# LIONS-EPFL/LEAF

Hardware: NVIDIA B200
Metric: leaf_candidates_scored_per_sec (higher is better)
Workload: dtype bf16

## Files before the change

include/leaf_b200.h:

```cpp
#ifndef LEAF_B200_H_
#define LEAF_B200_H_

#include <stdint.h>

#ifdef __cplusplus
extern "C" {
#endif

typedef enum {
  LEAF_OK = 0,
  LEAF_ERR_INVALID = -1,
  LEAF_ERR_CUDA = -2,
  LEAF_ERR_STATE = -3,
  LEAF_ERR_UNSUPPORTED = -4
} leaf_status_t;

typedef struct leaf_engine* leaf_handle_t;

enum { LEAF_ACT_GELU_ERF = 0, LEAF_ACT_QUICK_GELU = 1 };
enum { LEAF_OBJ_L2 = 0, LEAF_OBJ_NEGL2 = 1, LEAF_OBJ_SIM = 2, LEAF_OBJ_DISSIM = 3 };
enum { LEAF_CTX = 77, LEAF_SOT = 49406, LEAF_EOT = 49407, LEAF_VOCAB = 49408, LEAF_N_MERGES = 48894 };
enum { LEAF_MAX_CAPTION_BYTES = 1000, LEAF_MAX_CAPTION_BYTES_LONG = 3560 };

typedef struct {
// ... 68 lines not shown

typedef void (*leaf_backward_hook_t)(int32_t layer, void* user);
int leaf_set_backward_hook(leaf_handle_t h, leaf_backward_hook_t fn, void* user);
int leaf_set_sm_budget(leaf_handle_t h, int32_t n_sms);
int leaf_set_deterministic(leaf_handle_t h, int32_t on);

int leaf_adamw(leaf_handle_t h, float* params, const float* grads, float* exp_avg, float* exp_avg_sq, int64_t n,
               int64_t n_nodecay, float lr, float beta1, float beta2, float eps, float weight_decay, int32_t step,
               float grad_scale, void* stream);
int leaf_sumsq(leaf_handle_t h, const float* g, int64_t n, float* out, void* stream);
int leaf_scale(leaf_handle_t h, float* g, int64_t n, float s, void* stream);

int leaf_gemm_bf16(leaf_handle_t h, const void* A, const void* Bt, const float* bias, void* C,
                   int32_t M, int32_t N, int32_t K, int32_t epilogue, int32_t act, const int32_t* m_dev,
                   void* stream);
int leaf_gemm_bf16_mn(leaf_handle_t h, const void* A, const void* B, const float* bias, void* C, int32_t M, int32_t N,
                      int32_t K, int32_t epilogue, int32_t a_mn, void* stream);
int leaf_test_layernorm(leaf_handle_t h, const float* x, int32_t rows, const float* gamma, const float* beta, void* y,
                        void* stream);
int leaf_test_attention(leaf_handle_t h, const void* qkv, const int32_t* meta, int32_t N, void* out, void* stream);
int leaf_test_attention_bwd(leaf_handle_t h, const void* qkv, const void* o, const float* dout, const int32_t* meta, int32_t N,
                            int32_t T, void* dqkv, void* stream);
int leaf_set_prune_last(leaf_handle_t h, int32_t on);
int64_t leaf_launch_count(leaf_handle_t h, int32_t reset);
int64_t leaf_last_rows(leaf_handle_t h);
int leaf_set_timing(leaf_handle_t h, int32_t on);
double leaf_timing_ms(leaf_handle_t h, int32_t which, int32_t* launches);

#ifdef __cplusplus
}
// ... 3 lines not shown
```

leaf_b200/_native.py:

```python
import ctypes
import os

HERE = os.path.dirname(os.path.abspath(__file__))
LIB_PATH = os.environ.get("LEAF_B200_LIB") or os.path.join(HERE, "lib", "libleaf_b200.so")

c_int, c_void_p, c_float, c_i64 = ctypes.c_int32, ctypes.c_void_p, ctypes.c_float, ctypes.c_int64


class LeafCfg(ctypes.Structure):
    _fields_ = [("width", c_int), ("layers", c_int), ("heads", c_int), ("embed_dim", c_int), ("activation", c_int),
                ("ln_eps", c_float)]


class LeafLayerPtrs(ctypes.Structure):
    _fields_ = [(k, c_void_p) for k in (
        "ln1_w", "ln1_b", "in_proj_w", "in_proj_b", "q_w", "k_w", "v_w", "q_b", "k_b", "v_b", "out_w", "out_b",
        "ln2_w", "ln2_b", "fc1_w", "fc1_b", "fc2_w", "fc2_b")]


class LeafWeightPtrs(ctypes.Structure):
    _fields_ = [("token_embedding", c_void_p), ("positional_embedding", c_void_p), ("lnf_w", c_void_p),
                ("lnf_b", c_void_p), ("text_projection", c_void_p), ("projection_is_ew", c_int),
                ("layers", ctypes.POINTER(LeafLayerPtrs))]

# ... 17 lines not shown
    "leaf_encode": (c_int, [c_void_p, c_void_p, c_void_p, c_void_p, c_int, c_int, c_int, c_int, c_int, c_void_p, c_void_p]),
    "leaf_score": (c_int, [c_void_p, c_void_p, c_void_p, c_int, c_int, c_int, c_void_p, c_void_p, c_void_p, c_void_p]),
    "leaf_topk": (c_int, [c_void_p, c_void_p, c_void_p, c_int, c_int, c_void_p, c_void_p, c_void_p]),
    "leaf_train_reserve": (c_int, [c_void_p, c_int]),
    "leaf_forward_train": (c_int, [c_void_p, c_void_p, c_void_p, c_int, c_void_p, c_int, c_int, ctypes.POINTER(c_i64), c_void_p]),
    "leaf_backward": (c_int, [c_void_p, c_i64, c_void_p, c_int, ctypes.POINTER(LeafWeightPtrs), c_void_p]),
    "leaf_set_backward_hook": (c_int, [c_void_p, c_void_p, c_void_p]),
    "leaf_set_sm_budget": (c_int, [c_void_p, c_int]),
    "leaf_set_deterministic": (c_int, [c_void_p, c_int]),
    "leaf_adamw": (c_int, [c_void_p, c_void_p, c_void_p, c_void_p, c_void_p, c_i64, c_i64, ctypes.c_float, ctypes.c_float,
                           ctypes.c_float, ctypes.c_float, ctypes.c_float, c_int, ctypes.c_float, c_void_p]),
    "leaf_sumsq": (c_int, [c_void_p, c_void_p, c_i64, c_void_p, c_void_p]),
    "leaf_scale": (c_int, [c_void_p, c_void_p, c_i64, ctypes.c_float, c_void_p]),
    "leaf_gemm_bf16": (c_int, [c_void_p, c_void_p, c_void_p, c_void_p, c_void_p, c_int, c_int, c_int, c_int, c_int,
                               c_void_p, c_void_p]),
    "leaf_gemm_bf16_mn": (c_int, [c_void_p, c_void_p, c_void_p, c_void_p, c_void_p, c_int, c_int, c_int, c_int, c_int, c_void_p]),
    "leaf_test_layernorm": (c_int, [c_void_p, c_void_p, c_int, c_void_p, c_void_p, c_void_p, c_void_p]),
    "leaf_test_attention": (c_int, [c_void_p, c_void_p, c_void_p, c_int, c_void_p, c_void_p]),
    "leaf_test_attention_bwd": (c_int, [c_void_p, c_void_p, c_void_p, c_void_p, c_void_p, c_int, c_int, c_void_p, c_void_p]),
    "leaf_set_prune_last": (c_int, [c_void_p, c_int]),
    "leaf_launch_count": (c_i64, [c_void_p, c_int]),
    "leaf_last_rows": (c_i64, [c_void_p]),
    "leaf_set_timing": (c_int, [c_void_p, c_int]),
    "leaf_timing_ms": (ctypes.c_double, [c_void_p, c_int, ctypes.POINTER(c_int)]),
}

BACKWARD_HOOK = ctypes.CFUNCTYPE(None, c_int, c_void_p)

_lib = None

# ... 24 lines not shown
```

leaf_b200/csrc/engine.cu:

```cuda
#include <cuda.h>
#include <cuda_bf16.h>
#include <cuda_runtime.h>
#include <stdarg.h>
#include <stdint.h>
#include <stdio.h>
#include <stdlib.h>
#include <string.h>

#include <algorithm>
#include <map>
#include <string>
#include <tuple>
#include <vector>

#include "../../include/leaf_b200.h"
#include "gemm2_sm100.cuh"
#include "gemm_sm100.cuh"
#include "k1_tables_host.h"
#include "constrain_kernel.cuh"
#include "k1_tokenize.cuh"
#include "tower_kernels.cuh"
#include "attention2.cuh"
#include "train_kernels.cuh"

// ... 139 lines not shown
  cuuint64_t dims[2] = {static_cast<cuuint64_t>(mn_cols), static_cast<cuuint64_t>(k_rows)};
  cuuint64_t strides[1] = {static_cast<cuuint64_t>(pitch) * 2};
  cuuint32_t box[2] = {64, 64};
  cuuint32_t estr[2] = {1, 1};
  CUtensorMap m;
  CUresult r = e->encode_tiled(&m, CU_TENSOR_MAP_DATA_TYPE_BFLOAT16, 2, const_cast<void*>(ptr), dims, strides, box, estr,
                               CU_TENSOR_MAP_INTERLEAVE_NONE, CU_TENSOR_MAP_SWIZZLE_128B,
                               CU_TENSOR_MAP_L2_PROMOTION_L2_256B, CU_TENSOR_MAP_FLOAT_OOB_FILL_NONE);
  if (r != CUDA_SUCCESS) return fail(LEAF_ERR_CUDA, "cuTensorMapEncodeTiled (MN-major) failed (%d) rows=%ld cols=%ld", (int)r, k_rows, mn_cols);
  if (e->tmaps.size() > 4096) e->tmaps.clear();
  e->tmaps[key] = m;
  *out = m;
  return LEAF_OK;
}

static cudaEvent_t get_event(leaf_engine* e) {
  if (!e->event_pool.empty()) { cudaEvent_t ev = e->event_pool.back(); e->event_pool.pop_back(); return ev; }
  cudaEvent_t ev;
  cudaEventCreate(&ev);
  return ev;
}

struct TimedSpan {
  leaf_engine* e; cudaStream_t st; cudaEvent_t a = nullptr, b = nullptr; int cat;
  TimedSpan(leaf_engine* e_, int cat_, cudaStream_t st_) : e(e_), st(st_), cat(cat_) {
    if (e->timing) { a = get_event(e); b = get_event(e); cudaEventRecord(a, st); }
  }
  ~TimedSpan() {
    if (a) { cudaEventRecord(b, st); e->spans.push_back({a, b, cat}); }
  }
};

static int launch_gemm(leaf_engine* e, const __nv_bfloat16* A, long a_rows, const __nv_bfloat16* Bt, const float* bias,
                       void* C, int ldc, int M, int N, int K, int epi, int act, const int* m_dev, cudaStream_t st,
                       const __nv_bfloat16* delta = nullptr, int mn_major = 0, long a_pitch = 0, const float* res = nullptr,
                       void* C2 = nullptr, bool allow_split_k = false) {
  if (M <= 0 || N <= 0 || K <= 0) return fail(LEAF_ERR_INVALID, "GEMM shape %dx%dx%d", M, N, K);
  if (N % 8 != 0) return fail(LEAF_ERR_INVALID, "GEMM N (%d) must be a multiple of 8", N);
  CUtensorMap ta, tb;
  int a_box = a_rows < 128 ? static_cast<int>(a_rows) : 128;
  int b_box = N < 128 ? N : 128;
  int rc;
  if (mn_major & GEMM_A_MN) {
    if (M % 8 != 0) return fail(LEAF_ERR_INVALID, "MN-major GEMM M (%d) must be a multiple of 8", M);
    if ((rc = make_tmap_mn(e, A, K, M, a_pitch, &ta))) return rc;
    a_box = 128;
  } else if ((rc = make_tmap(e, A, a_rows, K, a_box, &ta))) return rc;
  if (mn_major & GEMM_B_MN) {
    if ((rc = make_tmap_mn(e, Bt, K, N, 0, &tb))) return rc;
    b_box = 128;
  } else if ((rc = make_tmap(e, Bt, N, K, b_box, &tb))) return rc;
  GemmParams p;
  p.mn_major = mn_major;
  p.res = res;
  p.C2 = C2;
  p.split_k = 1;
  p.ws = nullptr;
  p.cnt = nullptr;
  p.tx_bytes = static_cast<uint32_t>(a_box + b_box) * GEMM_BK * 2 * 2;
  p.M = M; p.m_dev = m_dev; p.N = N; p.K = K; p.bias = bias; p.C = C; p.ldc = ldc; p.act = act; p.delta = delta;
  const int m_tiles = (M + GEMM2_BM - 1) / GEMM2_BM, n_tiles = (N + GEMM_BN - 1) / GEMM_BN;
  long tiles = static_cast<long>(m_tiles) * n_tiles;
  const int pairs_cap = ((e->gemm_sm_budget > 0 && e->gemm_sm_budget < e->sm_count) ? e->gemm_sm_budget : e->sm_count) / 2;
  const bool det = e->deterministic && ((epi == EPI_BF16_ACTBWD && C2) || allow_split_k);
  const int split_pairs = det ? e->sm_count / 2 : pairs_cap;
  if (det) {
    if (!e->tw.det_ws) return fail(LEAF_ERR_STATE, "deterministic mode without its workspace (leaf_train_reserve)");
    p.ws = e->tw.det_ws;
    p.cnt = e->tw.det_cnt;
    if (epi == EPI_BF16_ACTBWD) {
      if (static_cast<size_t>((M + 31) / 32) * N > e->tw.det_ws_floats || static_cast<size_t>(n_tiles) * 4 > e->tw.det_cnt_ints)
// ... 5 lines not shown
    const int kblocks = (K + GEMM_BK - 1) / GEMM_BK;
    long best = ((tiles + split_pairs - 1) / split_pairs) * (kblocks + 3);
    for (int s = 2; s <= 8 && s <= kblocks; ++s) {
      const int kpb = (kblocks + s - 1) / s;
      const int s_eff = (kblocks + kpb - 1) / kpb;
      if (det && tiles * s_eff > 2L * split_pairs) continue;
      const long cost = ((tiles * s_eff + split_pairs - 1) / split_pairs) * (kpb + 3);
      if (cost < best) { best = cost; p.split_k = s_eff; }
    }
    if (det && p.split_k > 1 && (static_cast<size_t>(tiles) * p.split_k * GEMM2_BM * GEMM_BN > e->tw.det_ws_floats ||
                                 static_cast<size_t>(tiles) * 2 * EPI_WARPS > e->tw.det_cnt_ints))
      return fail(LEAF_ERR_STATE, "deterministic workspace too small for a %dx%d split-K product", M, N);
    tiles *= p.split_k;
    if (p.split_k > 1) epi = det ? EPI_F32_SPLITK_DET : EPI_F32_SPLITK;
  }
  TimedSpan span(e, (epi == EPI_F32_SPLITK || epi == EPI_F32_SPLITK_DET) ? 4 + EPI_F32_RESIDUAL :
                    (epi == EPI_BF16_ACTBWD || epi == EPI_BF16_ACTBWD_DET) ? 4 + EPI_F32 : (epi == EPI_F32_RESIDUAL && K > N) ? 8 : (epi == EPI_BF16 && K == N) ? 9 : 4 + epi, st);
  const int pairs = static_cast<int>(tiles < pairs_cap ? tiles : pairs_cap);
  cudaLaunchConfig_t cfg{};
  cfg.gridDim = dim3(2 * pairs);
  cfg.blockDim = dim3(GEMM_THREADS);
  cfg.dynamicSmemBytes = GEMM2_SMEM_BYTES;
  cfg.stream = st;
  cudaLaunchAttribute attr[2];
  attr[0].id = cudaLaunchAttributeClusterDimension;
  attr[0].val.clusterDim.x = 2; attr[0].val.clusterDim.y = 1; attr[0].val.clusterDim.z = 1;
  attr[1].id = cudaLaunchAttributeProgrammaticStreamSerialization;
  attr[1].val.programmaticStreamSerializationAllowed = 1;
  cfg.attrs = attr;
  cfg.numAttrs = e->pdl ? 2 : 1;
  switch (epi) {
    case EPI_BF16: CK(cudaLaunchKernelEx(&cfg, gemm2_bf16_tn_kernel<EPI_BF16>, ta, tb, p)); break;
    case EPI_BF16_ACT: CK(cudaLaunchKernelEx(&cfg, gemm2_bf16_tn_kernel<EPI_BF16_ACT>, ta, tb, p)); break;
    case EPI_F32_RESIDUAL: CK(cudaLaunchKernelEx(&cfg, gemm2_bf16_tn_kernel<EPI_F32_RESIDUAL>, ta, tb, p)); break;
    case EPI_F32: CK(cudaLaunchKernelEx(&cfg, gemm2_bf16_tn_kernel<EPI_F32>, ta, tb, p)); break;
    case EPI_F32_SPLITK: CK(cudaLaunchKernelEx(&cfg, gemm2_bf16_tn_kernel<EPI_F32_SPLITK>, ta, tb, p)); break;
    case EPI_BF16_ACTBWD: CK(cudaLaunchKernelEx(&cfg, gemm2_bf16_tn_kernel<EPI_BF16_ACTBWD>, ta, tb, p)); break;
    case EPI_F32_SPLITK_DET: CK(cudaLaunchKernelEx(&cfg, gemm2_bf16_tn_kernel<EPI_F32_SPLITK_DET>, ta, tb, p)); break;
    case EPI_BF16_ACTBWD_DET: CK(cudaLaunchKernelEx(&cfg, gemm2_bf16_tn_kernel<EPI_BF16_ACTBWD_DET>, ta, tb, p)); break;
    default: return fail(LEAF_ERR_INVALID, "unknown epilogue %d", epi);
  }
  e->launches++;
  CK(cudaGetLastError());
  return LEAF_OK;
}

extern "C" int leaf_create(const leaf_cfg_t* cfg, leaf_handle_t* out) {
  if (!cfg || !out) return fail(LEAF_ERR_INVALID, "null argument");
  if (cfg->width <= 0 || cfg->width % 128 != 0 || cfg->width > 2048)
    return fail(LEAF_ERR_INVALID, "width %d must be a multiple of 128 in (0, 2048]", cfg->width);
  if (cfg->heads <= 0 || cfg->width != cfg->heads * 64) return fail(LEAF_ERR_INVALID, "head_dim must be 64 (W=%d, H=%d)", cfg->width, cfg->heads);
  if (cfg->embed_dim <= 0 || cfg->embed_dim % 8 != 0) return fail(LEAF_ERR_INVALID, "embed_dim %d must be a multiple of 8", cfg->embed_dim);
  if (cfg->layers <= 0) return fail(LEAF_ERR_INVALID, "layers");
  int ndev = 0;
// ... 384 lines not shown
  if (!e || !score_a || !idx_out) return fail(LEAF_ERR_INVALID, "null argument");
  if (m <= 0 || k <= 0 || k > m) return fail(LEAF_ERR_INVALID, "top-k of m=%d, k=%d", m, k);
  const size_t smem = static_cast<size_t>(m) * 4;
  if (smem > 200 * 1024) return fail(LEAF_ERR_INVALID, "m=%d too large (max %d)", m, 200 * 1024 / 4);
  topk_kernel<<<1, 1024, smem, static_cast<cudaStream_t>(stream)>>>(score_a, score_b, m, k, idx_out, val_out);
  e->launches++;
  CK(cudaGetLastError());
  return LEAF_OK;
}

extern "C" int leaf_gemm_bf16(leaf_handle_t e, const void* A, const void* Bt, const float* bias, void* C, int32_t M, int32_t N,
                              int32_t K, int32_t epilogue, int32_t act, const int32_t* m_dev, void* stream) {
  if (!e || !A || !Bt || !C) return fail(LEAF_ERR_INVALID, "null argument");
  return launch_gemm(e, static_cast<const __nv_bfloat16*>(A), M, static_cast<const __nv_bfloat16*>(Bt), bias, C, N, M, N, K,
                     epilogue, act, m_dev, static_cast<cudaStream_t>(stream));
}

extern "C" int leaf_gemm_bf16_mn(leaf_handle_t e, const void* A, const void* B, const float* bias, void* C, int32_t M, int32_t N,
                                 int32_t K, int32_t epilogue, int32_t a_mn, void* stream) {
  if (!e || !A || !B || !C) return fail(LEAF_ERR_INVALID, "null argument");
  return launch_gemm(e, static_cast<const __nv_bfloat16*>(A), a_mn ? K : M, static_cast<const __nv_bfloat16*>(B), bias, C, N, M, N, K,
                     epilogue, 0, nullptr, static_cast<cudaStream_t>(stream), nullptr, GEMM_B_MN | (a_mn ? GEMM_A_MN : 0));
}

extern "C" int leaf_test_layernorm(leaf_handle_t e, const float* x, int32_t rows, const float* gamma, const float* beta, void* y,
                                   void* stream) {
  if (!e || !x || !gamma || !beta || !y || rows <= 0) return fail(LEAF_ERR_INVALID, "bad argument");
  return launch_layernorm(e, x, nullptr, rows, nullptr, gamma, beta, static_cast<__nv_bfloat16*>(y), static_cast<cudaStream_t>(stream));
}

// ... 469 lines not shown
```

leaf_b200/csrc/gemm2_sm100.cuh:

```cuda
#pragma once
#include "gemm_sm100.cuh"

namespace leaf {

constexpr int GEMM2_BM = 256;
constexpr int GEMM2_STAGES = 5;
constexpr uint32_t GEMM2_A_BYTES = 128 * GEMM_BK * 2;
constexpr uint32_t GEMM2_B_BYTES = 128 * GEMM_BK * 2;
constexpr uint32_t GEMM2_STAGE_BYTES = GEMM2_A_BYTES + GEMM2_B_BYTES;
constexpr uint32_t GEMM2_SMEM_BYTES = GEMM2_STAGES * GEMM2_STAGE_BYTES + EPI_WARPS * EPI_STAGE_BYTES + 1024  + 256 ;
constexpr int WARP_TMA = EPI_WARPS, WARP_MMA = EPI_WARPS + 1, WARP_TMEM = EPI_WARPS + 2;
constexpr uint32_t PEER_BIT_MASK = 0xFEFFFFFFu;

__device__ __forceinline__ uint32_t cluster_ctarank() {
  uint32_t r;
  asm volatile("mov.u32 %0, %%cluster_ctarank;" : "=r"(r));
  return r;
}
__device__ __forceinline__ bool elect_one() {
  uint32_t pred;
  asm volatile("{\n\t.reg .pred p;\n\telect.sync _|p, 0xffffffff;\n\tselp.u32 %0, 1, 0, p;\n\t}" : "=r"(pred));
  return pred != 0;
}
__device__ __forceinline__ void cluster_sync_all() {
  asm volatile("barrier.cluster.arrive.release.aligned;" ::: "memory");
// ... 19 lines not shown
      "tcgen05.mma.cta_group::2.kind::f16 [%0], %1, %2, %3, p;\n\t}"
      ::"r"(tmem_d), "l"(adesc), "l"(bdesc), "r"(idesc), "r"(accumulate)
      : "memory");
}
__device__ __forceinline__ void umma_commit_2sm(uint32_t bar) {
  asm volatile("tcgen05.commit.cta_group::2.mbarrier::arrive::one.shared::cluster.multicast::cluster.b64 [%0], %1;"
               ::"r"(bar), "h"(static_cast<uint16_t>(3)) : "memory");
}
__device__ __forceinline__ void mbar_arrive_leader(uint32_t bar_local) {
  asm volatile("mbarrier.arrive.shared::cluster.b64 _, [%0];" ::"r"(bar_local & PEER_BIT_MASK) : "memory");
}

template <int EPI>
__global__ void __launch_bounds__(GEMM_THREADS, 1)
gemm2_bf16_tn_kernel(const __grid_constant__ CUtensorMap tmap_a, const __grid_constant__ CUtensorMap tmap_b,
                     const GemmParams p) {
  extern __shared__ uint8_t smem_raw[];
  const uint32_t smem_base = (smem_u32(smem_raw) + 1023u) & ~1023u;
  const uint32_t bar_base = smem_base + GEMM2_STAGES * GEMM2_STAGE_BYTES + EPI_WARPS * EPI_STAGE_BYTES;
  auto full_bar = [&](int s) { return bar_base + 8u * s; };
  auto empty_bar = [&](int s) { return bar_base + 8u * (GEMM2_STAGES + s); };
  auto tfull_bar = [&](int s) { return bar_base + 8u * (2 * GEMM2_STAGES + s); };
  auto tempty_bar = [&](int s) { return bar_base + 8u * (2 * GEMM2_STAGES + 2 + s); };
  const uint32_t tmem_slot = bar_base + 8u * (2 * GEMM2_STAGES + 4);
  uint8_t* smem_gen = smem_raw + (smem_base - smem_u32(smem_raw));
  volatile uint32_t* tmem_slot_gen =
      reinterpret_cast<volatile uint32_t*>(smem_gen + GEMM2_STAGES * GEMM2_STAGE_BYTES + EPI_WARPS * EPI_STAGE_BYTES +
                                           8u * (2 * GEMM2_STAGES + 4));

  const int warp = threadIdx.x >> 5;
  const int lane = threadIdx.x & 31;
  const uint32_t rank = cluster_ctarank();
  const bool leader = rank == 0;
  const int pair = blockIdx.x >> 1, n_pairs = gridDim.x >> 1;
  const int M = p.m_dev ? min(*p.m_dev, p.M) : p.M;
  const int m_tiles = (M + GEMM2_BM - 1) / GEMM2_BM;
  const int n_tiles = (p.N + GEMM_BN - 1) / GEMM_BN;
  const int k_blocks = (p.K + GEMM_BK - 1) / GEMM_BK;
  const int split = ((EPI == EPI_F32_SPLITK || EPI == EPI_F32_SPLITK_DET) && p.split_k > 1) ? p.split_k : 1;
  const int kpb = (k_blocks + split - 1) / split;
  const int total_tiles = m_tiles * n_tiles * split;

  if (warp == WARP_TMA && lane == 0) {
    tma_prefetch_desc(&tmap_a);
    tma_prefetch_desc(&tmap_b);
  }
  if (warp == WARP_MMA && lane == 0) {
    for (int s = 0; s < GEMM2_STAGES; ++s) {
      mbar_init(full_bar(s), 1);
      mbar_init(empty_bar(s), 1);
    }
    for (int s = 0; s < 2; ++s) {
      mbar_init(tfull_bar(s), 1);
      mbar_init(tempty_bar(s), 2 * EPI_WARPS);
    }
    asm volatile("fence.mbarrier_init.release.cluster;" ::: "memory");
  }
  if (warp == WARP_TMEM) tmem_alloc_2sm(tmem_slot, 512);
  tc_fence_before();
  cluster_sync_all();
// ... 60 lines not shown
            umma_bf16_2sm(d_tmem, adesc + 2 * ak, bdesc + 2 * bk, idesc, 1u);
            umma_bf16_2sm(d_tmem, adesc + 3 * ak, bdesc + 3 * bk, idesc, 1u);
            umma_commit_2sm(empty_bar(stage));
            if (kb == kb1 - 1) umma_commit_2sm(tfull_bar(acc));
          }
          __syncwarp();
          if (++stage == GEMM2_STAGES) { stage = 0; phase ^= 1; }
        }
        if (++acc == 2) { acc = 0; acc_phase ^= 1; }
      }
    }
  } else if (warp < EPI_WARPS) {
    const int quad = warp & 3;
    const int part = warp >> 2;
    uint8_t* stage_buf = smem_gen + GEMM2_STAGES * GEMM2_STAGE_BYTES + warp * EPI_STAGE_BYTES;
    int acc = 0;
    uint32_t acc_phase = 0;
    for (int tile = pair; tile < total_tiles; tile += n_pairs) {
      const int mn = tile / split;
      const int m_blk = mn / n_tiles, n_blk = mn % n_tiles;
      mbar_wait(tfull_bar(acc), acc_phase);
      tc_fence_after();
      const int row0 = m_blk * GEMM2_BM + static_cast<int>(rank) * 128 + quad * 32;
#pragma unroll 1
      for (int c = 0; c < 64; c += 32) {
        const int col0 = n_blk * GEMM_BN + part * 64 + c;
        if (col0 >= p.N) break;
        ResidualRegs res;
        if (row0 < M) epilogue_load_residual<EPI>(p, res, lane, row0, col0, M);
        uint32_t v[32];
        const uint32_t taddr = tmem_base + (static_cast<uint32_t>(quad * 32) << 16) +
                               static_cast<uint32_t>(acc * GEMM_BN + part * 64 + c);
        tmem_ld32(taddr, v);
        tmem_ld_wait();
        if constexpr (EPI == EPI_F32_SPLITK_DET) {
          if (row0 < M) {
            float* w = p.ws + static_cast<size_t>(tile) * (GEMM2_BM * GEMM_BN) + ((rank * EPI_WARPS + warp) * 2 + (c >> 5)) * 1024 + lane;
#pragma unroll
            for (int j = 0; j < 32; ++j) w[j * 32] = __uint_as_float(v[j]);
          }
        } else {
          if (row0 < M) epilogue_chunk<EPI>(p, v, res, stage_buf, lane, row0, col0, M);
        }
      }
      tc_fence_before();
      __syncwarp();
      if (lane == 0) mbar_arrive_leader(tempty_bar(acc));
      if (++acc == 2) { acc = 0; acc_phase ^= 1; }
      if constexpr (EPI == EPI_F32_SPLITK_DET) {
        int* ctr = p.cnt + mn * (2 * EPI_WARPS) + rank * EPI_WARPS + warp;
// ... 41 lines not shown
          const int chunks = (M + 31) >> 5;
          if (old == chunks - 1) {
            __threadfence();
#pragma unroll 1
            for (int c = 0; c < 64; c += 32) {
              const int col = n_blk * GEMM_BN + part * 64 + c + lane;
              if (col < p.N) {
                reinterpret_cast<float*>(p.C2)[col] += ordered_sum<16>(p.ws + col, p.N, chunks);
              }
            }
            if (lane == 0) *ctr = 0;
          }
        }
      }
    }
  }

  tc_fence_before();
  cluster_sync_all();
  if (warp == WARP_TMEM) {
    tc_fence_after();
    tmem_dealloc_2sm(tmem_base, 512);
  }
}

}
```

leaf_b200/csrc/gemm_sm100.cuh:

```cuda
#pragma once
#include <cuda.h>
#include <cuda_bf16.h>
#include <cuda_runtime.h>
#include <stdint.h>

namespace leaf {

__device__ __forceinline__ void pdl_wait() { asm volatile("griddepcontrol.wait;" ::: "memory"); }
__device__ __forceinline__ void pdl_trigger() { asm volatile("griddepcontrol.launch_dependents;" ::: "memory"); }

constexpr int GEMM_BN = 256;
constexpr int GEMM_BK = 64;
constexpr int GEMM_UMMA_K = 16;

enum { EPI_BF16 = 0, EPI_BF16_ACT = 1, EPI_F32_RESIDUAL = 2, EPI_F32 = 3, EPI_F32_SPLITK = 4,
       EPI_BF16_ACTBWD = 5,
       EPI_F32_SPLITK_DET = 6, EPI_BF16_ACTBWD_DET = 7 };
enum { ACT_GELU_ERF = 0, ACT_QUICK_GELU = 1 };

struct GemmParams {
  int M;
  const int* m_dev;
  int N, K;
  const float* bias;
  void* C;
  const __nv_bfloat16* delta;
  const float* res;
  int ldc;
  int act;
  uint32_t tx_bytes;
  int mn_major;
  void* C2;
  int split_k;
  float* ws;
  int* cnt;
};
constexpr int GEMM_A_MN = 1, GEMM_B_MN = 2;
constexpr uint32_t GEMM_MN_LBO = 8192, GEMM_MN_SBO = 1024, GEMM_MN_KSTEP = 2048;

__device__ __forceinline__ uint32_t smem_u32(const void* p) {
  return static_cast<uint32_t>(__cvta_generic_to_shared(p));
}
__device__ __forceinline__ void mbar_init(uint32_t bar, uint32_t count) {
  asm volatile("mbarrier.init.shared::cta.b64 [%0], %1;" ::"r"(bar), "r"(count) : "memory");
}
__device__ __forceinline__ void mbar_arrive_expect_tx(uint32_t bar, uint32_t bytes) {
  asm volatile("mbarrier.arrive.expect_tx.shared::cta.b64 _, [%0], %1;" ::"r"(bar), "r"(bytes) : "memory");
}
__device__ __forceinline__ void mbar_arrive(uint32_t bar) {
  asm volatile("mbarrier.arrive.shared::cta.b64 _, [%0];" ::"r"(bar) : "memory");
// ... 11 lines not shown
        : "memory");
    if (done) return;
    if (it == 1024) t0 = clock64();
    if (it > 1024 && (it & 1023) == 0 && clock64() - t0 > 4000000000LL) __trap();
  }
}
__device__ __forceinline__ void tma_load_2d(uint32_t smem_dst, const CUtensorMap* tmap, uint32_t bar, int x, int y) {
  asm volatile(
      "cp.async.bulk.tensor.2d.shared::cluster.global.mbarrier::complete_tx::bytes [%0], [%1, {%3, %4}], [%2];"
      ::"r"(smem_dst), "l"(reinterpret_cast<uint64_t>(tmap)), "r"(bar), "r"(x), "r"(y)
      : "memory");
}
__device__ __forceinline__ void tma_prefetch_desc(const CUtensorMap* tmap) {
  asm volatile("prefetch.tensormap [%0];" ::"l"(reinterpret_cast<uint64_t>(tmap)) : "memory");
}
__device__ __forceinline__ void tc_fence_before() { asm volatile("tcgen05.fence::before_thread_sync;" ::: "memory"); }
__device__ __forceinline__ void tc_fence_after() { asm volatile("tcgen05.fence::after_thread_sync;" ::: "memory"); }
__device__ __forceinline__ void tmem_alloc(uint32_t smem_dst, uint32_t cols) {
  asm volatile("tcgen05.alloc.cta_group::1.sync.aligned.shared::cta.b32 [%0], %1;" ::"r"(smem_dst), "r"(cols) : "memory");
  asm volatile("tcgen05.relinquish_alloc_permit.cta_group::1.sync.aligned;" ::: "memory");
}
__device__ __forceinline__ void tmem_dealloc(uint32_t taddr, uint32_t cols) {
  asm volatile("tcgen05.dealloc.cta_group::1.sync.aligned.b32 %0, %1;" ::"r"(taddr), "r"(cols) : "memory");
}
__device__ __forceinline__ void umma_bf16(uint32_t tmem_d, uint64_t adesc, uint64_t bdesc, uint32_t idesc, uint32_t accumulate) {
  asm volatile(
      "{\n\t.reg .pred p;\n\t"
      "setp.ne.b32 p, %4, 0;\n\t"
      "tcgen05.mma.cta_group::1.kind::f16 [%0], %1, %2, %3, p;\n\t}"
      ::"r"(tmem_d), "l"(adesc), "l"(bdesc), "r"(idesc), "r"(accumulate)
// ... 72 lines not shown
__device__ __forceinline__ float quick_gelu(float x) {
  return x * fast_rcp(1.0f + fast_ex2(-1.702f * 1.4426950408889634f * x));
}
__device__ __forceinline__ float gelu_erf_grad(float x) {
  const float x2 = fminf(x * x, 36.0f);
  const float r = fmaf(x2, fmaf(x2, 0.0011236976601259265f, -0.10762115607988151f), -2.299969046114191f);
  const float cdf = fast_rcp(1.0f + fast_ex2(x * r));
  const float pdf = 0.3989422804014327f * fast_ex2(-0.5f * 1.4426950408889634f * x2);
  return fmaf(x, pdf, cdf);
}
__device__ __forceinline__ float quick_gelu_grad(float x) {
  const float s = fast_rcp(1.0f + fast_ex2(-1.702f * 1.4426950408889634f * x));
  return fmaf(1.702f * x * s, 1.0f - s, s);
}
constexpr int EPI_WARPS = 16;
constexpr int EPI_STAGE_BYTES = 32 * 80;
constexpr int GEMM_THREADS = 128 + 32 * EPI_WARPS;

struct ResidualRegs { float4 x[8]; };

template <int EPI>
__device__ __forceinline__ void epilogue_load_residual(const GemmParams& p, ResidualRegs& r, int lane, int row0, int col0, int M) {
  if (EPI != EPI_F32_RESIDUAL) return;
  const int c = lane & 3;
#pragma unroll
  for (int h = 0; h < 2; ++h) {
#pragma unroll
    for (int it = 0; it < 4; ++it) {
      const int row = row0 + it * 8 + (lane >> 2);
      const int col = col0 + h * 16 + c * 4;
      if (row < M && col < p.N)
        r.x[h * 4 + it] = *reinterpret_cast<const float4*>((p.res ? p.res : reinterpret_cast<const float*>(p.C)) + static_cast<size_t>(row) * p.ldc + col);
// ... 30 lines not shown
      pk.z = *reinterpret_cast<uint32_t*>(&t2);
      pk.w = *reinterpret_cast<uint32_t*>(&t3);
      *reinterpret_cast<uint4*>(stage + lane * 80 + q * 16) = pk;
    }
    __syncwarp();
    const bool col_ok = col0 + c * 8 < p.N;
#pragma unroll
    for (int it = 0; it < 4; ++it) {
      const int r = it * 8 + (lane >> 2);
      const uint4 pk = *reinterpret_cast<const uint4*>(stage + r * 80 + c * 16);
      if (col_ok && row0 + r < M)
        *reinterpret_cast<uint4*>(reinterpret_cast<__nv_bfloat16*>(dst) + static_cast<size_t>(row0 + r) * p.ldc + col0 + c * 8) = pk;
    }
    __syncwarp();
  };
  if (EPI == EPI_BF16_ACT) {
    if (p.C2) store_bf16(p.C2);
    if (p.act == ACT_QUICK_GELU) {
#pragma unroll
      for (int j = 0; j < 32; ++j) f[j] = quick_gelu(f[j]);
    } else {
#pragma unroll
      for (int j = 0; j < 32; ++j) f[j] = gelu_erf(f[j]);
    }
  }
  if (EPI == EPI_BF16_ACTBWD || EPI == EPI_BF16_ACTBWD_DET) {
#pragma unroll
    for (int it = 0; it < 4; ++it) {
      const int r = it * 8 + (lane >> 2);
      uint4 pk = make_uint4(0u, 0u, 0u, 0u);
      if (col0 + c * 8 < p.N && row0 + r < M)
        pk = *reinterpret_cast<const uint4*>(p.delta + static_cast<size_t>(row0 + r) * p.ldc + col0 + c * 8);
      *reinterpret_cast<uint4*>(stage + r * 80 + c * 16) = pk;
    }
    __syncwarp();
    const bool live = row0 + lane < M;
#pragma unroll
    for (int q = 0; q < 4; ++q) {
      const uint4 pk = *reinterpret_cast<const uint4*>(stage + lane * 80 + q * 16);
      const uint32_t w[4] = {pk.x, pk.y, pk.z, pk.w};
// ... 14 lines not shown
      for (int off = 16; off >= 1; off >>= 1) {
        const bool up = lane & off;
#pragma unroll
        for (int j = 0; j < off; ++j) {
          const float keep = up ? f[j + off] : f[j];
          const float send = up ? f[j] : f[j + off];
          f[j] = keep + __shfl_xor_sync(0xffffffffu, send, off);
        }
      }
      if (EPI == EPI_BF16_ACTBWD_DET) {
        if (col0 + lane < p.N) p.ws[static_cast<size_t>(row0 >> 5) * p.N + col0 + lane] = f[0];
      } else if (col0 + lane < p.N) {
        atomicAdd(reinterpret_cast<float*>(p.C2) + col0 + lane, f[0]);
      }
    }
  } else if (EPI == EPI_BF16 || EPI == EPI_BF16_ACT) {
    store_bf16(p.C);
  } else {
#pragma unroll
    for (int h = 0; h < 2; ++h) {
      uint2 dl[4];
      if (EPI == EPI_F32_RESIDUAL && p.delta) {
#pragma unroll
        for (int it = 0; it < 4; ++it) {
          const int row = row0 + it * 8 + (lane >> 2), col = col0 + h * 16 + c * 4;
          dl[it] = (row < M && col < p.N) ? *reinterpret_cast<const uint2*>(p.delta + static_cast<size_t>(row) * p.ldc + col)
                                          : make_uint2(0u, 0u);
        }
      }
#pragma unroll
      for (int q = 0; q < 4; ++q)
// ... 32 lines not shown
```

leaf_b200/engine.py:

```python
from __future__ import annotations

import ctypes
import os

import numpy as np
import torch

from . import _native
from ._native import LeafCfg, LeafLayerPtrs, LeafWeightPtrs, LeafError, check

HERE = os.path.dirname(os.path.abspath(__file__))
MERGES_BIN = os.path.join(HERE, "data", "clip_bpe_merges.bin")

CONTEXT_LENGTH = 77
OBJECTIVES = {"l2": 0, "negl2": 1, "sim": 2, "dissim": 3}
STATUS_ENTITY_DOMAIN, STATUS_NON_ASCII, STATUS_TOO_LONG = 1, 2, 4
MAX_CAPTION_BYTES = 1000
MAX_CAPTION_BYTES_LONG = 3560
MAX_CODE_POINT = 0x24F


def _ptr(t):
    return None if t is None else ctypes.c_void_p(t.data_ptr())

# ... 327 lines not shown
        val = torch.empty((k,), dtype=torch.float32, device=self.device)
        with torch.cuda.device(self.device):
            check(self._lib.leaf_topk(self._h, _ptr(score_a.contiguous()), _ptr(None if score_b is None else score_b.contiguous()), m, int(k),
                                      _ptr(idx), _ptr(val), _stream()))
        return idx, val

    def gemm(self, A, Bt, bias=None, epilogue=0, act=0, C=None, m_dev=None):
        M, K = A.shape
        N = Bt.shape[0]
        if C is None:
            C = torch.empty((M, N), dtype=torch.bfloat16 if epilogue in (0, 1) else torch.float32, device=A.device)
        with torch.cuda.device(self.device):
            check(self._lib.leaf_gemm_bf16(self._h, _ptr(A), _ptr(Bt), _ptr(bias), _ptr(C), M, N, K, epilogue, act, _ptr(m_dev), _stream()))
        return C

    def gemm_mn(self, A, B, bias=None, epilogue=3, C=None, a_mn=True):
        K, N = B.shape
        M = A.shape[1] if a_mn else A.shape[0]
        if C is None:
            C = torch.zeros((M, N), dtype=torch.bfloat16 if epilogue in (0, 1) else torch.float32, device=A.device)
        with torch.cuda.device(self.device):
            check(self._lib.leaf_gemm_bf16_mn(self._h, _ptr(A), _ptr(B), _ptr(bias), _ptr(C), M, N, K, epilogue, 1 if a_mn else 0,
                                              _stream()))
        return C

    def test_layernorm(self, x, gamma, beta):
        y = torch.empty(x.shape, dtype=torch.bfloat16, device=x.device)
        check(self._lib.leaf_test_layernorm(self._h, _ptr(x), x.shape[0], _ptr(gamma), _ptr(beta), _ptr(y), _stream()))
        return y

# ... 85 lines not shown
```

Before: 78480.

## Store GEMM epilogue outputs via TMA bulk tensor stores for act and f32 paths

```diff
diff --git a/include/leaf_b200.h b/include/leaf_b200.h
--- a/include/leaf_b200.h
+++ b/include/leaf_b200.h
@@ -106,6 +106,9 @@
 int leaf_gemm_bf16(leaf_handle_t h, const void* A, const void* Bt, const float* bias, void* C,
                    int32_t M, int32_t N, int32_t K, int32_t epilogue, int32_t act, const int32_t* m_dev,
                    void* stream);
+int leaf_gemm_bf16_ex(leaf_handle_t h, const void* A, const void* Bt, const float* bias, void* C, int32_t ldc, void* C2,
+                      const float* res, const void* delta, int32_t M, int32_t N, int32_t K, int32_t epilogue, int32_t act,
+                      const int32_t* m_dev, void* stream);
 int leaf_gemm_bf16_mn(leaf_handle_t h, const void* A, const void* B, const float* bias, void* C, int32_t M, int32_t N,
                       int32_t K, int32_t epilogue, int32_t a_mn, void* stream);
 int leaf_test_layernorm(leaf_handle_t h, const float* x, int32_t rows, const float* gamma, const float* beta, void* y,
diff --git a/leaf_b200/_native.py b/leaf_b200/_native.py
--- a/leaf_b200/_native.py
+++ b/leaf_b200/_native.py
@@ -55,6 +55,8 @@
     "leaf_scale": (c_int, [c_void_p, c_void_p, c_i64, ctypes.c_float, c_void_p]),
     "leaf_gemm_bf16": (c_int, [c_void_p, c_void_p, c_void_p, c_void_p, c_void_p, c_int, c_int, c_int, c_int, c_int,
                                c_void_p, c_void_p]),
+    "leaf_gemm_bf16_ex": (c_int, [c_void_p, c_void_p, c_void_p, c_void_p, c_void_p, c_int, c_void_p, c_void_p, c_void_p, c_int,
+                                  c_int, c_int, c_int, c_int, c_void_p, c_void_p]),
     "leaf_gemm_bf16_mn": (c_int, [c_void_p, c_void_p, c_void_p, c_void_p, c_void_p, c_int, c_int, c_int, c_int, c_int, c_void_p]),
     "leaf_test_layernorm": (c_int, [c_void_p, c_void_p, c_int, c_void_p, c_void_p, c_void_p, c_void_p]),
     "leaf_test_attention": (c_int, [c_void_p, c_void_p, c_void_p, c_int, c_void_p, c_void_p]),
diff --git a/leaf_b200/csrc/engine.cu b/leaf_b200/csrc/engine.cu
--- a/leaf_b200/csrc/engine.cu
+++ b/leaf_b200/csrc/engine.cu
@@ -177,6 +177,27 @@
   return LEAF_OK;
 }
 
+static int make_tmap_out(leaf_engine* e, const void* ptr, long rows, long cols, long pitch, int elem_bytes, CUtensorMap* out) {
+  auto key = std::make_tuple(ptr, rows, cols, static_cast<int>(0x40000000L | (static_cast<long>(elem_bytes) << 24) | pitch));
+  auto it = e->tmaps.find(key);
+  if (it != e->tmaps.end()) { *out = it->second; return LEAF_OK; }
+  if ((reinterpret_cast<uintptr_t>(ptr) & 15) || (pitch * elem_bytes) % 16 != 0 || pitch >= (1L << 24))
+    return fail(LEAF_ERR_INVALID, "GEMM output must be 16-byte aligned with a 16-byte multiple row pitch (pitch %ld)", pitch);
+  cuuint64_t dims[2] = {static_cast<cuuint64_t>(cols), static_cast<cuuint64_t>(rows)};
+  cuuint64_t strides[1] = {static_cast<cuuint64_t>(pitch) * elem_bytes};
+  cuuint32_t box[2] = {static_cast<cuuint32_t>(64 / elem_bytes), 32};
+  cuuint32_t estr[2] = {1, 1};
+  CUtensorMap m;
+  CUresult r = e->encode_tiled(&m, elem_bytes == 2 ? CU_TENSOR_MAP_DATA_TYPE_BFLOAT16 : CU_TENSOR_MAP_DATA_TYPE_FLOAT32, 2,
+                               const_cast<void*>(ptr), dims, strides, box, estr, CU_TENSOR_MAP_INTERLEAVE_NONE,
+                               CU_TENSOR_MAP_SWIZZLE_64B, CU_TENSOR_MAP_L2_PROMOTION_L2_128B, CU_TENSOR_MAP_FLOAT_OOB_FILL_NONE);
+  if (r != CUDA_SUCCESS) return fail(LEAF_ERR_CUDA, "cuTensorMapEncodeTiled (output) failed (%d) rows=%ld cols=%ld", (int)r, rows, cols);
+  if (e->tmaps.size() > 4096) e->tmaps.clear();
+  e->tmaps[key] = m;
+  *out = m;
+  return LEAF_OK;
+}
+
 static cudaEvent_t get_event(leaf_engine* e) {
   if (!e->event_pool.empty()) { cudaEvent_t ev = e->event_pool.back(); e->event_pool.pop_back(); return ev; }
   cudaEvent_t ev;
@@ -200,6 +221,15 @@
                        void* C2 = nullptr, bool allow_split_k = false) {
   if (M <= 0 || N <= 0 || K <= 0) return fail(LEAF_ERR_INVALID, "GEMM shape %dx%dx%d", M, N, K);
   if (N % 8 != 0) return fail(LEAF_ERR_INVALID, "GEMM N (%d) must be a multiple of 8", N);
+  {
+    const bool bf16_out = epi == EPI_BF16 || epi == EPI_BF16_ACT || epi == EPI_BF16_ACTBWD;
+    auto rows_aligned = [&](const void* ptr, int elem_bytes) {
+      return !ptr || ((reinterpret_cast<uintptr_t>(ptr) & 15) == 0 && (static_cast<long>(ldc) * elem_bytes) % 16 == 0);
+    };
+    if (ldc < N || !rows_aligned(C, bf16_out ? 2 : 4) || (epi == EPI_BF16_ACT && !rows_aligned(C2, 2)) ||
+        !rows_aligned(res, 4) || !rows_aligned(delta, 2))
+      return fail(LEAF_ERR_INVALID, "GEMM output rows must be 16-byte aligned (ldc %d, N %d)", ldc, N);
+  }
   CUtensorMap ta, tb;
   int a_box = a_rows < 128 ? static_cast<int>(a_rows) : 128;
   int b_box = N < 128 ? N : 128;
@@ -218,6 +248,7 @@
   p.res = res;
   p.C2 = C2;
   p.split_k = 1;
+  p.c_tma = 0;
   p.ws = nullptr;
   p.cnt = nullptr;
   p.tx_bytes = static_cast<uint32_t>(a_box + b_box) * GEMM_BK * 2 * 2;
@@ -253,6 +284,12 @@
     tiles *= p.split_k;
     if (p.split_k > 1) epi = det ? EPI_F32_SPLITK_DET : EPI_F32_SPLITK;
   }
+  CUtensorMap tc{}, tc2{};
+  if ((epi == EPI_BF16_ACT || epi == EPI_F32) && M >= 32) {
+    if ((rc = make_tmap_out(e, C, M, N, ldc, epi == EPI_F32 ? 4 : 2, &tc))) return rc;
+    if (epi == EPI_BF16_ACT && C2 && (rc = make_tmap_out(e, C2, M, N, ldc, 2, &tc2))) return rc;
+    p.c_tma = 1;
+  }
   TimedSpan span(e, (epi == EPI_F32_SPLITK || epi == EPI_F32_SPLITK_DET) ? 4 + EPI_F32_RESIDUAL :
                     (epi == EPI_BF16_ACTBWD || epi == EPI_BF16_ACTBWD_DET) ? 4 + EPI_F32 : (epi == EPI_F32_RESIDUAL && K > N) ? 8 : (epi == EPI_BF16 && K == N) ? 9 : 4 + epi, st);
   const int pairs = static_cast<int>(tiles < pairs_cap ? tiles : pairs_cap);
@@ -269,14 +306,14 @@
   cfg.attrs = attr;
   cfg.numAttrs = e->pdl ? 2 : 1;
   switch (epi) {
-    case EPI_BF16: CK(cudaLaunchKernelEx(&cfg, gemm2_bf16_tn_kernel<EPI_BF16>, ta, tb, p)); break;
-    case EPI_BF16_ACT: CK(cudaLaunchKernelEx(&cfg, gemm2_bf16_tn_kernel<EPI_BF16_ACT>, ta, tb, p)); break;
-    case EPI_F32_RESIDUAL: CK(cudaLaunchKernelEx(&cfg, gemm2_bf16_tn_kernel<EPI_F32_RESIDUAL>, ta, tb, p)); break;
-    case EPI_F32: CK(cudaLaunchKernelEx(&cfg, gemm2_bf16_tn_kernel<EPI_F32>, ta, tb, p)); break;
-    case EPI_F32_SPLITK: CK(cudaLaunchKernelEx(&cfg, gemm2_bf16_tn_kernel<EPI_F32_SPLITK>, ta, tb, p)); break;
-    case EPI_BF16_ACTBWD: CK(cudaLaunchKernelEx(&cfg, gemm2_bf16_tn_kernel<EPI_BF16_ACTBWD>, ta, tb, p)); break;
-    case EPI_F32_SPLITK_DET: CK(cudaLaunchKernelEx(&cfg, gemm2_bf16_tn_kernel<EPI_F32_SPLITK_DET>, ta, tb, p)); break;
-    case EPI_BF16_ACTBWD_DET: CK(cudaLaunchKernelEx(&cfg, gemm2_bf16_tn_kernel<EPI_BF16_ACTBWD_DET>, ta, tb, p)); break;
+    case EPI_BF16: CK(cudaLaunchKernelEx(&cfg, gemm2_bf16_tn_kernel<EPI_BF16>, ta, tb, tc, tc2, p)); break;
+    case EPI_BF16_ACT: CK(cudaLaunchKernelEx(&cfg, gemm2_bf16_tn_kernel<EPI_BF16_ACT>, ta, tb, tc, tc2, p)); break;
+    case EPI_F32_RESIDUAL: CK(cudaLaunchKernelEx(&cfg, gemm2_bf16_tn_kernel<EPI_F32_RESIDUAL>, ta, tb, tc, tc2, p)); break;
+    case EPI_F32: CK(cudaLaunchKernelEx(&cfg, gemm2_bf16_tn_kernel<EPI_F32>, ta, tb, tc, tc2, p)); break;
+    case EPI_F32_SPLITK: CK(cudaLaunchKernelEx(&cfg, gemm2_bf16_tn_kernel<EPI_F32_SPLITK>, ta, tb, tc, tc2, p)); break;
+    case EPI_BF16_ACTBWD: CK(cudaLaunchKernelEx(&cfg, gemm2_bf16_tn_kernel<EPI_BF16_ACTBWD>, ta, tb, tc, tc2, p)); break;
+    case EPI_F32_SPLITK_DET: CK(cudaLaunchKernelEx(&cfg, gemm2_bf16_tn_kernel<EPI_F32_SPLITK_DET>, ta, tb, tc, tc2, p)); break;
+    case EPI_BF16_ACTBWD_DET: CK(cudaLaunchKernelEx(&cfg, gemm2_bf16_tn_kernel<EPI_BF16_ACTBWD_DET>, ta, tb, tc, tc2, p)); break;
     default: return fail(LEAF_ERR_INVALID, "unknown epilogue %d", epi);
   }
   e->launches++;
@@ -691,6 +728,17 @@
   if (!e || !A || !Bt || !C) return fail(LEAF_ERR_INVALID, "null argument");
   return launch_gemm(e, static_cast<const __nv_bfloat16*>(A), M, static_cast<const __nv_bfloat16*>(Bt), bias, C, N, M, N, K,
                      epilogue, act, m_dev, static_cast<cudaStream_t>(stream));
+}
+
+extern "C" int leaf_gemm_bf16_ex(leaf_handle_t e, const void* A, const void* Bt, const float* bias, void* C, int32_t ldc, void* C2,
+                                 const float* res, const void* delta, int32_t M, int32_t N, int32_t K, int32_t epilogue, int32_t act,
+                                 const int32_t* m_dev, void* stream) {
+  if (!e || !A || !Bt || !C) return fail(LEAF_ERR_INVALID, "null argument");
+  if (ldc < N) return fail(LEAF_ERR_INVALID, "ldc %d < N %d", ldc, N);
+  if ((C2 && epilogue != EPI_BF16_ACT) || ((res || delta) && epilogue != EPI_F32_RESIDUAL))
+    return fail(LEAF_ERR_INVALID, "C2 goes with epilogue 1, res and delta with epilogue 2");
+  return launch_gemm(e, static_cast<const __nv_bfloat16*>(A), M, static_cast<const __nv_bfloat16*>(Bt), bias, C, ldc, M, N, K,
+                     epilogue, act, m_dev, static_cast<cudaStream_t>(stream), static_cast<const __nv_bfloat16*>(delta), 0, 0, res, C2);
 }
 
 extern "C" int leaf_gemm_bf16_mn(leaf_handle_t e, const void* A, const void* B, const float* bias, void* C, int32_t M, int32_t N,
diff --git a/leaf_b200/csrc/gemm2_sm100.cuh b/leaf_b200/csrc/gemm2_sm100.cuh
--- a/leaf_b200/csrc/gemm2_sm100.cuh
+++ b/leaf_b200/csrc/gemm2_sm100.cuh
@@ -9,6 +9,9 @@
 constexpr uint32_t GEMM2_B_BYTES = 128 * GEMM_BK * 2;
 constexpr uint32_t GEMM2_STAGE_BYTES = GEMM2_A_BYTES + GEMM2_B_BYTES;
 constexpr uint32_t GEMM2_SMEM_BYTES = GEMM2_STAGES * GEMM2_STAGE_BYTES + EPI_WARPS * EPI_STAGE_BYTES + 1024  + 256 ;
+static_assert(GEMM2_SMEM_BYTES <= 227 * 1024, "shared memory of one block");
+template <int EPI>
+__host__ __device__ constexpr bool epi_tma() { return EPI == EPI_BF16_ACT || EPI == EPI_F32; }
 constexpr int WARP_TMA = EPI_WARPS, WARP_MMA = EPI_WARPS + 1, WARP_TMEM = EPI_WARPS + 2;
 constexpr uint32_t PEER_BIT_MASK = 0xFEFFFFFFu;
 
@@ -58,6 +61,7 @@
 template <int EPI>
 __global__ void __launch_bounds__(GEMM_THREADS, 1)
 gemm2_bf16_tn_kernel(const __grid_constant__ CUtensorMap tmap_a, const __grid_constant__ CUtensorMap tmap_b,
+                     const __grid_constant__ CUtensorMap tmap_c, const __grid_constant__ CUtensorMap tmap_c2,
                      const GemmParams p) {
   extern __shared__ uint8_t smem_raw[];
   const uint32_t smem_base = (smem_u32(smem_raw) + 1023u) & ~1023u;
@@ -88,6 +92,10 @@
   if (warp == WARP_TMA && lane == 0) {
     tma_prefetch_desc(&tmap_a);
     tma_prefetch_desc(&tmap_b);
+    if (epi_tma<EPI>() && p.c_tma) {
+      tma_prefetch_desc(&tmap_c);
+      if (EPI == EPI_BF16_ACT && p.C2) tma_prefetch_desc(&tmap_c2);
+    }
   }
   if (warp == WARP_MMA && lane == 0) {
     for (int s = 0; s < GEMM2_STAGES; ++s) {
@@ -178,6 +186,8 @@
     const int quad = warp & 3;
     const int part = warp >> 2;
     uint8_t* stage_buf = smem_gen + GEMM2_STAGES * GEMM2_STAGE_BYTES + warp * EPI_STAGE_BYTES;
+    const uint32_t box0 = smem_base + GEMM2_STAGES * GEMM2_STAGE_BYTES + warp * EPI_STAGE_BYTES;
+    int box = 0;
     int acc = 0;
     uint32_t acc_phase = 0;
     for (int tile = pair; tile < total_tiles; tile += n_pairs) {
@@ -186,6 +196,7 @@
       mbar_wait(tfull_bar(acc), acc_phase);
       tc_fence_after();
       const int row0 = m_blk * GEMM2_BM + static_cast<int>(rank) * 128 + quad * 32;
+      const bool full = epi_tma<EPI>() && p.c_tma && row0 + 32 <= M;
 #pragma unroll 1
       for (int c = 0; c < 64; c += 32) {
         const int col0 = n_blk * GEMM_BN + part * 64 + c;
@@ -197,7 +208,10 @@
                                static_cast<uint32_t>(acc * GEMM_BN + part * 64 + c);
         tmem_ld32(taddr, v);
         tmem_ld_wait();
-        if constexpr (EPI == EPI_F32_SPLITK_DET) {
+        if constexpr (epi_tma<EPI>()) {
+          if (row0 < M)
+            epilogue_chunk_tma<EPI>(p, v, &tmap_c, &tmap_c2, box0, stage_buf, box, lane, row0, col0, M, full);
+        } else if constexpr (EPI == EPI_F32_SPLITK_DET) {
           if (row0 < M) {
             float* w = p.ws + static_cast<size_t>(tile) * (GEMM2_BM * GEMM_BN) + ((rank * EPI_WARPS + warp) * 2 + (c >> 5)) * 1024 + lane;
 #pragma unroll
@@ -269,6 +283,7 @@
         }
       }
     }
+    if (epi_tma<EPI>() && lane == 0) bulk_wait_all();
   }
 
   tc_fence_before();
diff --git a/leaf_b200/csrc/gemm_sm100.cuh b/leaf_b200/csrc/gemm_sm100.cuh
--- a/leaf_b200/csrc/gemm_sm100.cuh
+++ b/leaf_b200/csrc/gemm_sm100.cuh
@@ -34,6 +34,7 @@
   int split_k;
   float* ws;
   int* cnt;
+  int c_tma;
 };
 constexpr int GEMM_A_MN = 1, GEMM_B_MN = 2;
 constexpr uint32_t GEMM_MN_LBO = 8192, GEMM_MN_SBO = 1024, GEMM_MN_KSTEP = 2048;
@@ -75,6 +76,16 @@
 __device__ __forceinline__ void tma_prefetch_desc(const CUtensorMap* tmap) {
   asm volatile("prefetch.tensormap [%0];" ::"l"(reinterpret_cast<uint64_t>(tmap)) : "memory");
 }
+__device__ __forceinline__ void tma_store_2d(const CUtensorMap* tmap, uint32_t smem_src, int x, int y) {
+  asm volatile("cp.async.bulk.tensor.2d.global.shared::cta.bulk_group [%0, {%2, %3}], [%1];"
+               ::"l"(reinterpret_cast<uint64_t>(tmap)), "r"(smem_src), "r"(x), "r"(y)
+               : "memory");
+}
+__device__ __forceinline__ void bulk_commit() { asm volatile("cp.async.bulk.commit_group;" ::: "memory"); }
+template <int N>
+__device__ __forceinline__ void bulk_wait_read() { asm volatile("cp.async.bulk.wait_group.read %0;" ::"n"(N) : "memory"); }
+__device__ __forceinline__ void bulk_wait_all() { asm volatile("cp.async.bulk.wait_group 0;" ::: "memory"); }
+__device__ __forceinline__ void fence_proxy_async_smem() { asm volatile("fence.proxy.async.shared::cta;" ::: "memory"); }
 __device__ __forceinline__ void tc_fence_before() { asm volatile("tcgen05.fence::before_thread_sync;" ::: "memory"); }
 __device__ __forceinline__ void tc_fence_after() { asm volatile("tcgen05.fence::after_thread_sync;" ::: "memory"); }
 __device__ __forceinline__ void tmem_alloc(uint32_t smem_dst, uint32_t cols) {
@@ -177,8 +188,89 @@
   return fmaf(1.702f * x * s, 1.0f - s, s);
 }
 constexpr int EPI_WARPS = 16;
-constexpr int EPI_STAGE_BYTES = 32 * 80;
 constexpr int GEMM_THREADS = 128 + 32 * EPI_WARPS;
+constexpr int EPI_BOX_BYTES = 32 * 64;
+constexpr int EPI_STAGE_BYTES = 2 * EPI_BOX_BYTES;
+static_assert(32 * 80 <= EPI_STAGE_BYTES, "padded staging buffer");
+
+__device__ __forceinline__ uint32_t box64_off(int r, int q) {
+  return static_cast<uint32_t>(r * 64 + ((q ^ ((r >> 1) & 3)) << 4));
+}
+
+template <int EPI>
+__device__ __forceinline__ void epilogue_chunk_tma(const GemmParams& p, const uint32_t* v, const CUtensorMap* tmap_c,
+                                                   const CUtensorMap* tmap_c2, uint32_t box0, uint8_t* box0_gen, int& box,
+                                                   int lane, int row0, int col0, int M, bool full) {
+  float f[32];
+#pragma unroll
+  for (int j = 0; j < 32; ++j) f[j] = __uint_as_float(v[j]);
+  if (p.bias) {
+#pragma unroll
+    for (int j = 0; j < 32; j += 4) {
+      if (col0 + j < p.N) {
+        const float4 b = __ldg(reinterpret_cast<const float4*>(p.bias + col0 + j));
+        f[j] += b.x; f[j + 1] += b.y; f[j + 2] += b.z; f[j + 3] += b.w;
+      }
+    }
+  }
+  const bool row_ok = row0 + lane < M;
+  auto store_row = [&](const uint4* pk, void* dst, int elem_bytes, const CUtensorMap* tmap, int x) {
+    if (full) {
+      if (lane == 0) bulk_wait_read<1>();
+      __syncwarp();
+      uint8_t* b = box0_gen + box * EPI_BOX_BYTES;
+#pragma unroll
+      for (int q = 0; q < 4; ++q) *reinterpret_cast<uint4*>(b + box64_off(lane, q)) = pk[q];
+      fence_proxy_async_smem();
+      __syncwarp();
+      if (lane == 0) {
+        tma_store_2d(tmap, box0 + box * EPI_BOX_BYTES, x, row0);
+        bulk_commit();
+      }
+      box ^= 1;
+    } else if (row_ok) {
+      uint8_t* out = reinterpret_cast<uint8_t*>(dst) + (static_cast<size_t>(row0 + lane) * p.ldc + x) * elem_bytes;
+      const int per_q = 16 / elem_bytes;
+#pragma unroll
+      for (int q = 0; q < 4; ++q)
+        if (x + per_q * q < p.N) *reinterpret_cast<uint4*>(out + 16 * q) = pk[q];
+    }
+  };
+  if (EPI == EPI_BF16_ACT) {
+    auto store_bf16 = [&](void* dst, const CUtensorMap* tmap) {
+      uint4 pk[4];
+#pragma unroll
+      for (int q = 0; q < 4; ++q) {
+        __nv_bfloat162 t0 = __floats2bfloat162_rn(f[8 * q], f[8 * q + 1]);
+        __nv_bfloat162 t1 = __floats2bfloat162_rn(f[8 * q + 2], f[8 * q + 3]);
+        __nv_bfloat162 t2 = __floats2bfloat162_rn(f[8 * q + 4], f[8 * q + 5]);
+        __nv_bfloat162 t3 = __floats2bfloat162_rn(f[8 * q + 6], f[8 * q + 7]);
+        pk[q] = make_uint4(*reinterpret_cast<uint32_t*>(&t0), *reinterpret_cast<uint32_t*>(&t1),
+                           *reinterpret_cast<uint32_t*>(&t2), *reinterpret_cast<uint32_t*>(&t3));
+      }
+      store_row(pk, dst, 2, tmap, col0);
+    };
+    if (p.C2) store_bf16(p.C2, tmap_c2);
+    if (p.act == ACT_QUICK_GELU) {
+#pragma unroll
+      for (int j = 0; j < 32; ++j) f[j] = quick_gelu(f[j]);
+    } else {
+#pragma unroll
+      for (int j = 0; j < 32; ++j) f[j] = gelu_erf(f[j]);
+    }
+    store_bf16(p.C, tmap_c);
+  } else {
+#pragma unroll
+    for (int h = 0; h < 2; ++h) {
+      uint4 pk[4];
+#pragma unroll
+      for (int q = 0; q < 4; ++q)
+        pk[q] = make_uint4(__float_as_uint(f[16 * h + 4 * q]), __float_as_uint(f[16 * h + 4 * q + 1]),
+                           __float_as_uint(f[16 * h + 4 * q + 2]), __float_as_uint(f[16 * h + 4 * q + 3]));
+      store_row(pk, p.C, 4, tmap_c, col0 + 16 * h);
+    }
+  }
+}
 
 struct ResidualRegs { float4 x[8]; };
 
@@ -239,16 +331,6 @@
     }
     __syncwarp();
   };
-  if (EPI == EPI_BF16_ACT) {
-    if (p.C2) store_bf16(p.C2);
-    if (p.act == ACT_QUICK_GELU) {
-#pragma unroll
-      for (int j = 0; j < 32; ++j) f[j] = quick_gelu(f[j]);
-    } else {
-#pragma unroll
-      for (int j = 0; j < 32; ++j) f[j] = gelu_erf(f[j]);
-    }
-  }
   if (EPI == EPI_BF16_ACTBWD || EPI == EPI_BF16_ACTBWD_DET) {
 #pragma unroll
     for (int it = 0; it < 4; ++it) {
@@ -293,7 +375,7 @@
         atomicAdd(reinterpret_cast<float*>(p.C2) + col0 + lane, f[0]);
       }
     }
-  } else if (EPI == EPI_BF16 || EPI == EPI_BF16_ACT) {
+  } else if (EPI == EPI_BF16) {
     store_bf16(p.C);
   } else {
 #pragma unroll
diff --git a/leaf_b200/engine.py b/leaf_b200/engine.py
--- a/leaf_b200/engine.py
+++ b/leaf_b200/engine.py
@@ -365,6 +365,16 @@
             check(self._lib.leaf_gemm_bf16(self._h, _ptr(A), _ptr(Bt), _ptr(bias), _ptr(C), M, N, K, epilogue, act, _ptr(m_dev), _stream()))
         return C
 
+    def gemm_ex(self, A, Bt, bias, epilogue, C, act=0, C2=None, res=None, delta=None, m_dev=None):
+        M, K = A.shape
+        N = Bt.shape[0]
+        for t in (C, C2, res, delta):
+            assert t is None or (t.shape[0] >= M and t.shape[1] == N and t.stride(1) == 1 and t.stride(0) == C.stride(0))
+        with torch.cuda.device(self.device):
+            check(self._lib.leaf_gemm_bf16_ex(self._h, _ptr(A), _ptr(Bt), _ptr(bias), _ptr(C), C.stride(0), _ptr(C2), _ptr(res),
+                                              _ptr(delta), M, N, K, epilogue, act, _ptr(m_dev), _stream()))
+        return C
+
     def gemm_mn(self, A, B, bias=None, epilogue=3, C=None, a_mn=True):
         K, N = B.shape
         M = A.shape[1] if a_mn else A.shape[0]
```

Measured after the change: 79330 (median of 6 runs). 1.1% higher.
